# homopolymer/RAMBL

Measured on AMD Instinct MI355X. Metric: reads/sec into POA (150bp, ~1.5k-node graph), higher is better.
Workload: dtype f64

## Files before the change

### rambl_amd/csrc/sc_kernels.hip

```cpp
#include <hip/hip_runtime.h>
#include <math.h>
#include <stdint.h>
#include <stdlib.h>

#include "sc_device.hpp"

namespace sc {

#define SC_GLOBAL __attribute__((address_space(1)))
#define SC_LDS __attribute__((address_space(3)))

constexpr int LDS_TOTAL = 160 * 1024 - 256;
constexpr int LDS_SMALL = 18 * 1024;
constexpr int LDS_BIG = LDS_TOTAL - LDS_SMALL;
static_assert(LDS_SMALL >= (int)(sizeof(double) * 2 * MAXS + sizeof(StrainParam) * MAXS + sizeof(unsigned) * MAXS * KMAX + sizeof(int) * 6 * MAXS + 64), "LDS_SMALL");
static_assert(LDS_BIG >= (int)(sizeof(double) * MAXS * 64), "LDS_BIG");

template <int CTRL, int ROW_MASK, int BANK_MASK, bool BOUND>
__device__ __forceinline__ double dpp_f64(double v) {
    int lo = __double2loint(v), hi = __double2hiint(v);
    lo = __builtin_amdgcn_update_dpp(0, lo, CTRL, ROW_MASK, BANK_MASK, BOUND);
    hi = __builtin_amdgcn_update_dpp(0, hi, CTRL, ROW_MASK, BANK_MASK, BOUND);
    return __hiloint2double(hi, lo);
}
// ... 98 lines not shown
#pragma unroll
    for (int i = 0; i < NPL; i++) {
        const int s = lane * NPL + i;
        x[i] = -INFINITY;
        if (s < S) {
            const double* row = job.ll + (long)s_slot[s] * job.ll_stride;
            double v = hr ? row[rid] : 0.0;
            if (hu) v += row[uid];
            x[i] = v;
            m = fmax(m, v);
        }
    }
    for (int d = 1; d < 64; d <<= 1) m = fmax(m, __shfl_xor(m, d));
    const bool flag = !(m >= -600.0);
    double w[NPL], pair = 0;
#pragma unroll
    for (int i = 0; i < NPL; i++) {
        const int s = lane * NPL + i;
        w[i] = (s < S) ? a[i] * exp(x[i] - m) : 0.0;
        pair += w[i];
    }
    const double incl = wave_scan_incl(pair);
    const double T = readlane_f64(incl, 63);
    const double tgt = u * T;
    const double lo = tgt - DRAW_EPS64 * T, hi = tgt + DRAW_EPS64 * T;
    bool ok = (T > 0.0) && (T < 1.0e300) && !flag;
    int c;
    if (NPL == 1) {
        const unsigned long long mlo = __ballot(incl >= lo), mhi = __ballot(incl >= hi);
        ok = ok && (mlo == mhi) && (mlo != 0ull);
        c = ok ? (int)__builtin_ctzll(mlo) : 0;
    } else {
        const double E = wave_shr1(incl);
        const double c0 = E + w[0], c1 = E + pair;
        const unsigned long long m0lo = __ballot(c0 >= lo), m0hi = __ballot(c0 >= hi);
        const unsigned long long m1lo = __ballot(c1 >= lo), m1hi = __ballot(c1 >= hi);
        ok = ok && (m0lo == m0hi) && (m1lo == m1hi) && (m1lo != 0ull);
        const int l1 = ok ? (int)__builtin_ctzll(m1lo) : 0;
        c = 2 * l1 + (((m0lo >> l1) & 1ull) ? 0 : 1);
    }
    if (!ok) {
#pragma unroll
        for (int i = 0; i < NPL; i++) { int s = lane * NPL + i; if (s < S) s_a[s] = a[i]; }
        __builtin_amdgcn_wave_barrier();
        int cc = 0;
        if (lane == 0) cc = exact_draw(job, s_slot, s_a, s_p, S, rid, uid, u);
        c = __builtin_amdgcn_readfirstlane(cc);
        __builtin_amdgcn_wave_barrier();
        c |= 0x100;
    }
    return c;
}

typedef float f4v __attribute__((ext_vector_type(4)));
typedef float f2v __attribute__((ext_vector_type(2)));
typedef int i4v __attribute__((ext_vector_type(4)));
typedef unsigned u4v __attribute__((ext_vector_type(4)));

__device__ __forceinline__ float fma_rn(float a, float b, float c) {
    float d;
    asm("v_fma_f32 %0, %1, %2, %3" : "=v"(d) : "v"(a), "v"(b), "v"(c));
    return d;
}
__device__ __forceinline__ f2v pk_sub(f2v a, f2v b) {
    f2v d;
    asm("v_pk_add_f32 %0, %1, %2 neg_lo:[0,1] neg_hi:[0,1]" : "=v"(d) : "v"(a), "v"(b));
    return d;
}
__device__ __forceinline__ unsigned min3_u32(unsigned m, unsigned x, unsigned y) {
    unsigned d;
    asm("v_min3_u32 %0, %1, %2, %3" : "=v"(d) : "v"(m), "v"(x), "v"(y));
    return d;
}
template <int QP> __device__ __forceinline__ float quad_f32(float v) {
    return __int_as_float(__builtin_amdgcn_update_dpp(0, __float_as_int(v), QP, 0xF, 0xF, true));
}
template <int QP> __device__ __forceinline__ int quad_i32(int v) {
    return __builtin_amdgcn_update_dpp(0, v, QP, 0xF, 0xF, true);
}
__device__ __forceinline__ void lds_barrier() { asm volatile("s_waitcnt lgkmcnt(0)\n\ts_barrier" ::: "memory"); }

constexpr int UWIN = 1024;
#ifdef SC_CHAIN_PROF
__device__ unsigned long long g_chain_prof[12];
#define CHAIN_STAMP(k) do { if (wv == 0) { const unsigned long long t_ = clock64(); prof[k] += t_ - tprev; tprev = t_; } } while (0)
#define CHAIN_STAMP_W(k) do { asm volatile("s_waitcnt lgkmcnt(0)" ::: "memory"); CHAIN_STAMP(k); } while (0)
#else
#define CHAIN_STAMP(k) do {} while (0)
#define CHAIN_STAMP_W(k) do {} while (0)
#endif

template <int NQ, bool ROWS_LDS, int NW, class JD>
__device__ __forceinline__ void urn_chain_q(const JD& job, const LevelHdr& h, const StrainParam* s_sp, LevelResult* __restrict__ R,
                                            const int* s_slot, volatile double* s_a, volatile double* s_p, unsigned* s_kf,
                                            const float* s_a0f, int* s_x, float* s_uwin, const float* rows_lds, int stride, int tid) {
    constexpr int SPL = 4 * NQ, SP = 16 * NQ;
    constexpr int NPLC = SP > 64 ? 2 : 1;
    constexpr float EPSW = (float)(SP + 16) * 1.5e-7f;
    const int lane = tid & 63, wv = __builtin_amdgcn_readfirstlane(tid >> 6), k = lane & 3, pos = wv * 16 + (lane >> 2);
    const int S = h.S, Q = h.Q, n = h.n_sweeps, e0 = h.e0;
    const int Sm1 = S - 1;
    const int total = n * Q;
    const SlowArgs sa{job.qent, job.quid, job.ent_rid, job.ll, job.ll_stride, job.has};
    const SC_GLOBAL double* Ustream = (const SC_GLOBAL double*)job.U;
    const SC_GLOBAL float* Uf = (const SC_GLOBAL float*)job.Uf;
    const SC_GLOBAL float* rows_g = (const SC_GLOBAL float*)job.tabLf;
    SC_GLOBAL unsigned char* dlog = (SC_GLOBAL unsigned char*)job.dlog;
    auto ld4 = [&](int idx) __attribute__((always_inline)) -> f4v {
        return ROWS_LDS ? *(const f4v*)(rows_lds + idx) : *(const SC_GLOBAL f4v*)(rows_g + idx);
    };
    auto ld1 = [&](int idx) __attribute__((always_inline)) -> float { return ROWS_LDS ? rows_lds[idx] : rows_g[idx]; };

    const int cbase = k * SPL;
    const float m0 = k > 0 ? 1.0f : 0.0f, m1 = k > 1 ? 1.0f : 0.0f;
    const float posf = (float)pos + 1.0e-37f;
    double a0m[NPLC];
#pragma unroll
    for (int i = 0; i < NPLC; i++) { const int s = lane * NPLC + i; a0m[i] = (s < S) ? s_sp[s].a0 : 0.0; }
    f4v a0q[NQ];
#pragma unroll
    for (int g = 0; g < NQ; g++) a0q[g] = *(const f4v*)(s_a0f + cbase + 4 * g);
    unsigned long long n_exact = 0, n_slow = 0, n_pass = 0;
    const unsigned long long clk0 = clock64(), wall0 = wall_clock64();

    int ulo = 0;
    bool upf = false;
    f4v ux0 = 0.0f, ux1 = 0.0f;
    if (wv == 0) {
#pragma unroll
        for (int j = 0; j < UWIN / 256; j++) *(f4v*)(s_uwin + 256 * j + 4 * lane) = *(const SC_GLOBAL f4v*)(Uf + 256 * j + 4 * lane);
    }
    __syncthreads();

    int t = 0;
    int ro = (pos % Q) * stride;
    const int wrap = Q * stride;
    int upos = pos;
    f4v L[NQ];
    float uf = 0.0f, llast = 0.0f;
    auto issue_loads = [&]() __attribute__((always_inline)) {
#pragma unroll
        for (int g = 0; g < NQ; g++) L[g] = ld4(ro + cbase + 4 * g);
        llast = ld1(ro + Sm1);
        uf = s_uwin[upos];
    };
    if (total > 0) issue_loads();
#ifdef SC_CHAIN_PROF
    unsigned long long prof[9] = {0, 0, 0, 0, 0, 0, 0, 0, 0}, tprev = clock64();
#endif
#pragma unroll 1
    while (t < total) {
        asm volatile("" ::: "memory");
        n_pass++;
        float loc[SPL];
        float run = 0.0f;
        u4v kq[NQ];
#pragma unroll
        for (int g = 0; g < NQ; g++) kq[g] = *(const u4v*)(s_kf + cbase + 4 * g);
        const unsigned klast = s_kf[Sm1];
        const float a0last = s_a0f[Sm1];
#pragma unroll
        for (int g = 0; g < NQ; g++) {
            const u4v kk = kq[g];
            const f4v av = a0q[g] + f4v{(float)kk.x, (float)kk.y, (float)kk.z, (float)kk.w};
            loc[4 * g + 0] = run = (g == 0) ? av.x * L[g].x : fma_rn(av.x, L[g].x, run);
            loc[4 * g + 1] = run = fma_rn(av.y, L[g].y, run);
            loc[4 * g + 2] = run = fma_rn(av.z, L[g].z, run);
            loc[4 * g + 3] = run = fma_rn(av.w, L[g].w, run);
        }
        const float alast = a0last + (float)klast;
        CHAIN_STAMP(0);
        const float i1 = fmaf(quad_f32<0x90>(run), m0, run);
        const float i2 = fmaf(quad_f32<0x40>(i1), m1, i1);
        const float off = i2 - run;
        const float T = quad_f32<0xFF>(i2);
        const float tgt = uf * T;
        const float tb = tgt - off;
        const f2v tb2 = {tb, tb};
        unsigned w = 0;
        unsigned up = 0x7f800000u, dn = 0x7f800000u;
#pragma unroll
        for (int j = 0; j < SPL; j += 2) {
            const f2v lc = {loc[j], loc[j + 1]};
            const f2v d = pk_sub(lc, tb2);
            const f2v e = pk_sub(tb2, lc);
            w = __builtin_amdgcn_alignbit(w, __float_as_uint(d.x), 31);
            w = __builtin_amdgcn_alignbit(w, __float_as_uint(d.y), 31);
            up = min3_u32(up, __float_as_uint(d.x), __float_as_uint(d.y));
            dn = min3_u32(dn, __float_as_uint(e.x), __float_as_uint(e.y));
        }
        const float alt = tgt - (T - alast * llast);
        const float epsT = EPSW * T;
        const float lim_up = fmaf(uf + 0x1p-22f, posf, epsT);
        const float lim_dn = fmaf((1.0f + 0x1p-22f) - uf, posf, epsT);
        const bool okl = (__uint_as_float(dn) >= lim_dn) && ((__uint_as_float(up) >= lim_up) || (alt >= lim_dn));
        const unsigned long long F = ~__ballot(okl);
        const int fpos = F ? 16 * wv + ((int)__builtin_ctzll(F) >> 2) : 16 * NW;
        if (lane == 0) s_x[wv] = fpos;
        int c = __popc(w);
        c += quad_i32<0xB1>(c);
        c += quad_i32<0x4E>(c);
        c = min(c, Sm1);
        CHAIN_STAMP(1);
        lds_barrier();
        const int rem = total - t;
        int adv = 16 * NW;
#pragma unroll
        for (int j = 0; j < NW / 4; j++) {
            const i4v xf = *(const i4v*)(s_x + 4 * j);
            adv = min(adv, min(min(xf.x, xf.y), min(xf.z, xf.w)));
        }
        adv = adv < rem ? adv : rem;
        CHAIN_STAMP(2);
        if (adv == 0) {
            if (wv == 0) {
                const double u = Ustream[t];
                double ad[NPLC];
#pragma unroll
                for (int i = 0; i < NPLC; i++) { const int s = lane * NPLC + i; ad[i] = a0m[i] + (double)((s < S) ? s_kf[s] : 0u); }
                const int qi = __builtin_amdgcn_readfirstlane(ro) / stride;
                const int cc = slow_draw<NPLC>(sa, s_slot, s_a, s_p, ad[0], NPLC > 1 ? ad[NPLC - 1] : 0.0, S, qi, e0, u, lane);
                n_slow++;
                n_exact += (cc >> 8) & 1;
                c = cc & 0xFF;
            }
            adv = 1;
        }
        const bool acc = (pos < adv) && (k == 0);
        SC_GLOBAL unsigned char* const lg = dlog + (t + pos);
        t += adv;
        if (t >= total) {
            if (acc) { __hip_atomic_fetch_add(&s_kf[c], 1u, __ATOMIC_RELAXED, __HIP_MEMORY_SCOPE_WORKGROUP); *lg = (unsigned char)c; }
            break;
        }
        if (Q >= 16 * NW) {
            const unsigned r1 = (unsigned)(ro + adv * stride);
            const unsigned r2 = r1 - (unsigned)wrap;
            ro = (int)(r1 < r2 ? r1 : r2);
        } else {
            ro = ((ro / stride + adv) % Q) * stride;
        }
        upos = (upos + adv) & (UWIN - 1);
        if (wv == 0) {
            if (!upf && t >= ulo + UWIN / 4) {
                ux0 = *(const SC_GLOBAL f4v*)(Uf + ulo + UWIN + 4 * lane);
                ux1 = *(const SC_GLOBAL f4v*)(Uf + ulo + UWIN + 256 + 4 * lane);
                upf = true;
            }
            if (t >= ulo + UWIN / 2) {
                *(f4v*)(s_uwin + ((ulo & (UWIN - 1)) + 4 * lane)) = ux0;
                *(f4v*)(s_uwin + ((ulo & (UWIN - 1)) + 256 + 4 * lane)) = ux1;
                ulo += UWIN / 2;
                upf = false;
            }
        }
        CHAIN_STAMP(3);
        issue_loads();
        CHAIN_STAMP_W(6);
        if (acc) __hip_atomic_fetch_add(&s_kf[c], 1u, __ATOMIC_RELAXED, __HIP_MEMORY_SCOPE_WORKGROUP);
        CHAIN_STAMP_W(7);
        if (acc) *lg = (unsigned char)c;
        CHAIN_STAMP_W(8);
        lds_barrier();
        CHAIN_STAMP(4);
    }
#ifdef SC_CHAIN_PROF
    if (tid == 0) { for (int i = 0; i < 9; i++) if (i != 5) atomicAdd(&g_chain_prof[i], prof[i]); atomicAdd(&g_chain_prof[5], n_pass); }
#endif
    asm volatile("s_waitcnt vmcnt(0)" ::: "memory");
    __syncthreads();
    if (wv == 0) {
#pragma unroll
        for (int i = 0; i < NPLC; i++) {
            const int s = lane * NPLC + i;
            if (s < S) { R->abund[s] = a0m[i] + (double)s_kf[s]; R->kdraw[s] = s_kf[s]; }
        }
        if (lane == 0) {
            R->n_draws = (unsigned long long)total; R->n_exact = n_exact; R->n_slow = n_slow; R->n_pass = n_pass;
            R->chain_cycles = clock64() - clk0; R->chain_wall = wall_clock64() - wall0;
        }
    }
}

template <class JD>
__device__ __forceinline__ void draw_log_counts(const JD& job, const LevelHdr& h, unsigned* s_cnt, int tid, int nt) {
    const int Q = h.Q, n = h.n_sweeps;
    if (Q <= 0 || n <= 0) return;
    __builtin_amdgcn_fence(__ATOMIC_ACQUIRE, "agent");
    const SC_GLOBAL unsigned char* dlog = (const SC_GLOBAL unsigned char*)job.dlog;
    const int G = Q < nt ? min(nt / Q, n) : 1;
    const int per = (n + G - 1) / G;
    for (int idx = tid; idx < Q * G; idx += nt) {
        const int q = idx % Q, j0 = (idx / Q) * per, j1 = min(j0 + per, n);
        const int sym = job.qcode[q];
        if (sym >= KMAX || j0 >= j1) continue;
        const SC_GLOBAL unsigned char* p = dlog + (j0 * Q + q);
        int cur = 0;
        unsigned run = 0;
        auto count = [&](int c) __attribute__((always_inline)) {
            if (c != cur) {
                if (run) __hip_atomic_fetch_add(&s_cnt[cur * KMAX + sym], run, __ATOMIC_RELAXED, __HIP_MEMORY_SCOPE_WORKGROUP);
                cur = c; run = 0;
            }
            run++;
        };
        int j = j0;
        for (; j + 8 <= j1; j += 8, p += 8 * Q) {
            int c[8];
#pragma unroll
            for (int i = 0; i < 8; i++) c[i] = p[i * Q] & (MAXS - 1);
#pragma unroll
            for (int i = 0; i < 8; i++) count(c[i]);
        }
        for (; j < j1; j++, p += Q) count(*p & (MAXS - 1));
        if (run) __hip_atomic_fetch_add(&s_cnt[cur * KMAX + sym], run, __ATOMIC_RELAXED, __HIP_MEMORY_SCOPE_WORKGROUP);
    }
}

template <int NW>
__device__ __forceinline__ void urn_chain_shadow(const LevelHdr& h, const int* s_x) {
    const int total = h.n_sweeps * h.Q;
    __syncthreads();
    int t = 0;
#pragma unroll 1
    while (t < total) {
        lds_barrier();
        int adv = 16 * NW;
#pragma unroll
        for (int j = 0; j < NW / 4; j++) {
            const i4v xf = *(const volatile i4v*)(s_x + 4 * j);
            adv = min(adv, min(min(xf.x, xf.y), min(xf.z, xf.w)));
        }
        const int rem = total - t;
        adv = adv < rem ? adv : rem;
        if (adv == 0) adv = 1;
        t += adv;
        if (t >= total) break;
        lds_barrier();
    }
    __syncthreads();
}

enum { LV_COPIES_DONE = 1, LV_ITEMS_DONE = 2, LV_HAS_DONE = 4, LV_HARD_DONE = 8 };
typedef const __attribute__((address_space(4))) JobDev KJob;

__global__ __launch_bounds__(256) void k_level_copy(JobDev job, const LevelParams* __restrict__ P) {
    const int c = blockIdx.y;
    const double2* src = reinterpret_cast<const double2*>(job.ll + (long)P->copy_src[c] * job.ll_stride);
    double2* dst = reinterpret_cast<double2*>(job.ll + (long)P->copy_dst[c] * job.ll_stride);
    const int n2 = (job.n_reads + 1) >> 1;
    for (int i = blockIdx.x * blockDim.x + threadIdx.x; i < n2; i += gridDim.x * blockDim.x) dst[i] = src[i];
}

__global__ __launch_bounds__(256) void k_level_update(JobDev job, LevelHdr h, const LevelParams* __restrict__ P) {
    __shared__ double s_row[MAXS * KMAX];
    __shared__ double s_diag[MAXS * KMAX];
    __shared__ int s_slot[MAXS], s_lab[MAXS];
    const int tid = threadIdx.x;
    const int S = h.S, K = job.K, e0 = h.e0, Rn = h.e1 - h.e0, codeN = job.code_N;
    for (int s = tid; s < S; s += blockDim.x) { s_slot[s] = P->sp[s].slot; s_lab[s] = job.labels[P->sp[s].lab_off]; }
    __syncthreads();
    for (int i = tid; i < S * KMAX; i += blockDim.x) {
        const int sx = i / KMAX, b = i % KMAX, a = s_lab[sx];
        const double* lp = P->lpt + (long)sx * K * K;
        s_row[i] = (a < K && b < K) ? lp[a * K + b] : 0.0;
        s_diag[i] = (b < K) ? lp[b * K + b] : 0.0;
    }
    __syncthreads();
    const long total = (long)S * Rn;
    const long stride = job.ll_stride;
    for (long idx = (long)blockIdx.x * blockDim.x + tid; idx < total; idx += (long)gridDim.x * blockDim.x) {
        const int sx = (int)(idx / Rn), e = e0 + (int)(idx % Rn);
        const int rid = job.ent_rid[e];
        const int b = job.labels[job.ent_lab_off[e]];
        const bool fresh = job.ent_first[e] && !job.has[rid];
        if (sx == 0) job.isnew[e - e0] = fresh ? 1 : 0;
        int a = s_lab[sx];
        const bool wild = (a == codeN);
        if (wild) a = b;
        const double val = (a < K && b < K) ? (wild ? s_diag[sx * KMAX + b] : s_row[sx * KMAX + b]) : __longlong_as_double(0x7ff8000000000000ll);
        double* cell = job.ll + (long)s_slot[sx] * stride + rid;
        *cell = fresh ? val : (*cell + val);
    }
}

__global__ __launch_bounds__(256) void k_level_has(JobDev job, LevelHdr h) {
    const int Rn = h.e1 - h.e0;
    for (int r = blockIdx.x * blockDim.x + threadIdx.x; r < Rn; r += gridDim.x * blockDim.x) job.has[job.ent_rid[h.e0 + r]] = 1;
}

__global__ __launch_bounds__(256) void k_hard_slots(JobDev job, LevelHdr h) {
    const int e0 = h.e0, Rn = h.e1 - h.e0;
    for (int r = blockIdx.x * blockDim.x + threadIdx.x; r < Rn; r += gridDim.x * blockDim.x) {
        const int e = e0 + r;
        const int rid = job.ent_rid[e], cn = job.ent_cn[e];
        const int qb = job.ent_qoff[e];
        const int mb = job.mate_ptr[rid], mn = job.mate_ptr[rid + 1] - mb;
        const uint8_t code = (job.ent_lab_len[e] == 1) ? job.labels[job.ent_lab_off[e]] : (uint8_t)0xFF;
        for (int i = 0; i < cn; i++) {
            const int k = cn - 1 - i;
            job.qent[qb + i] = r;
            job.quid[qb + i] = (k < mn) ? job.mate_idx[mb + k] : -1;
            job.qcode[qb + i] = code;
        }
    }
}
__global__ __launch_bounds__(256) void k_hard_mates(JobDev job, LevelHdr h, const LevelParams* __restrict__ P) {
    const long stride = job.ll_stride;
    for (int q = blockIdx.x * blockDim.x + threadIdx.x; q < h.Q; q += gridDim.x * blockDim.x) {
        const int uid = job.quid[q];
// ... 176 lines not shown
            }
        }
    } else if (!h.has_dups) {
        const long total = (long)S * Rn;
        for (long idx = tid; idx < total; idx += nt) item((int)(idx / Rn), (int)(idx % Rn));
    } else {
        if (tid < S) for (int r = 0; r < Rn; r++) item(tid, r);
    }
    if (h.done & LV_HAS_DONE) { __syncthreads(); return; }
    __syncthreads();
    for (int r = tid; r < Rn; r += nt) job.has[job.ent_rid[e0 + r]] = 1;
    __syncthreads();
}

template <bool BARRIER = true, class JD>
__device__ __forceinline__ void phase_slots(const JD& job, const LevelHdr& h, int tid, int nt) {
    const int e0 = h.e0, Rn = h.e1 - h.e0;
    for (int r = tid; r < Rn; r += nt) {
        const int e = e0 + r;
        const int rid = job.ent_rid[e], cn = job.ent_cn[e];
        const int qb = job.ent_qoff[e];
        const int mb = job.mate_ptr[rid], mn = job.mate_ptr[rid + 1] - mb;
        const uint8_t code = (job.ent_lab_len[e] == 1) ? job.labels[job.ent_lab_off[e]] : (uint8_t)0xFF;
        for (int i = 0; i < cn; i++) {
            const int k = cn - 1 - i;
            const int uid = (k < mn) ? job.mate_idx[mb + k] : -1;
            job.qent[qb + i] = r;
            job.quid[qb + i] = uid;
            job.qcode[qb + i] = code;
        }
    }
    if (BARRIER) __syncthreads();
}

__device__ __forceinline__ void finish_level(const LevelHdr& h, LevelResult* __restrict__ R, unsigned long long wall0, int tid) {
    __threadfence_system();
    __syncthreads();
    if (tid == 0) {
        R->level_wall = wall_clock64() - wall0;
        R->xcc = (int)(__builtin_amdgcn_s_getreg(20 | (3 << 11)) & 0xF);
        R->xcc = (int)(__builtin_amdgcn_s_getreg(20 | (3 << 11)) & 0xF);
        __hip_atomic_store(&R->seq, h.seq, __ATOMIC_RELEASE, __HIP_MEMORY_SCOPE_SYSTEM);
    }
}

__device__ __forceinline__ float exp_weight(double y) {
    if (y < -104.0) return 0.0f;
    const double k = rint(y * 1.4426950408889634);
    double r = fma(k, -0.693147180559945286, y);
    r = fma(k, -2.3190468138462996e-17, r);
    const float e = __builtin_amdgcn_exp2f((float)r * 1.44269504f);
    const double kc = fmax(k, -300.0);
    return (y == y) ? ldexpf(e, (int)kc) : __int_as_float(0x7fc00000);
}

__host__ __device__ inline int chain_w_stride(int S) {
    const int s4 = (S + 1 + 3) & ~3;
    return (s4 & 4) ? s4 : s4 + 4;
}

struct LevelLds {
    double* s_a; double* s_p; unsigned* s_cnt; int* s_slot; unsigned* s_kf; float* s_a0f; int* s_x; int* s_copy; int* s_lab;
    StrainParam* s_sp; unsigned char* s_big;
};
__device__ __forceinline__ LevelLds level_lds(unsigned char* raw) {
    LevelLds l;
    l.s_a = reinterpret_cast<double*>(raw);
    l.s_p = l.s_a + MAXS;
    l.s_sp = reinterpret_cast<StrainParam*>(l.s_p + MAXS);
    l.s_cnt = reinterpret_cast<unsigned*>(l.s_sp + MAXS);
    l.s_slot = reinterpret_cast<int*>(l.s_cnt + MAXS * KMAX);
    l.s_kf = reinterpret_cast<unsigned*>(l.s_slot + MAXS);
    l.s_a0f = reinterpret_cast<float*>(l.s_kf + MAXS);
    l.s_copy = reinterpret_cast<int*>(l.s_a0f + MAXS);
    l.s_lab = l.s_copy + 2 * MAXS;
    l.s_x = l.s_lab + MAXS;
    l.s_big = raw + LDS_SMALL;
    return l;
}

constexpr int CHAINW_ROWS_BYTES = LDS_BIG - UWIN * 4;
constexpr int CHAIN_THREADS = 512;
constexpr int chain_nw(int nb) { return nb <= 2 ? 8 : 4; }
template <class IT>
__device__ __forceinline__ LevelHdr load_hdr(const IT& it) {
    LevelHdr h;
    h.mode = it.h.mode; h.S = it.h.S; h.e0 = it.h.e0; h.e1 = it.h.e1; h.has_dups = it.h.has_dups; h.any_multi = it.h.any_multi;
    h.Q = it.h.Q; h.n_sweeps = it.h.n_sweeps; h.n_copy = it.h.n_copy; h.do_update = it.h.do_update; h.done = it.h.done;
    h.copy_n = it.h.copy_n; h.seq = it.h.seq;
    return h;
}
template <int NB, bool ROWS_LDS, bool STAY, class IT>
__device__ __forceinline__ void level_sample_body(const IT& it, unsigned char* s_raw) {
    const unsigned long long wall0 = wall_clock64();
    const LevelHdr h = load_hdr(it);
    KJob& job = *(KJob*)it.job;
    const LevelParams* __restrict__ P = it.P;
    LevelResult* __restrict__ R = it.R;
    const LevelLds l = level_lds(s_raw);
    float* s_uwin = reinterpret_cast<float*>(l.s_big);
    float* s_rows = s_uwin + UWIN;
    const int tid = threadIdx.x;
    int nt = blockDim.x;
    const int S = h.S, Q = h.Q, e0 = h.e0, Rn = h.e1 - h.e0;
    const int stride = chain_w_stride(S);
    const bool upd = h.do_update && Rn > 0;
    stage_params(h, P, l.s_sp, l.s_copy, reinterpret_cast<double*>(l.s_big), upd && !(h.done & LV_ITEMS_DONE), job.K * job.K, tid, nt);
    for (int i = tid; i < MAXS * KMAX; i += nt) l.s_cnt[i] = 0;
    if (tid == 0) { R->error = 0; R->n_draws = 0; R->n_exact = 0; R->n_slow = 0; R->n_pass = 0; R->chain_cycles = 0; R->chain_wall = 0; }
    __syncthreads();
    if (tid == 0) R->phase_ticks[0] = (unsigned)(wall_clock64() - wall0);
    if (tid < MAXS) {
        l.s_slot[tid] = tid < S ? l.s_sp[tid].slot : 0;
        l.s_kf[tid] = 0u;
        l.s_a0f[tid] = tid < S ? (float)l.s_sp[tid].a0 : 0.0f;
        l.s_lab[tid] = tid < S ? (int)job.labels[l.s_sp[tid].lab_off] : 0;
    }
    phase_copies(job, h, l.s_copy, tid, nt);
    if (tid == 0) R->phase_ticks[1] = (unsigned)(wall_clock64() - wall0);
    if (upd) {
        phase_slots<false>(job, h, tid, nt);
        phase_update(job, h, l.s_sp, l.s_lab, reinterpret_cast<const double*>(l.s_big), tid, nt);
    }
    if (tid == 0) R->phase_ticks[2] = (unsigned)(wall_clock64() - wall0);
    if (!upd) phase_slots(job, h, tid, nt);
    if (tid == 0) R->phase_ticks[3] = (unsigned)(wall_clock64() - wall0);

    {
        constexpr int SR = (NB <= 2) ? 16 * NB : 16;
        const long lstride = job.ll_stride;
        SC_GLOBAL float* rows_g = (SC_GLOBAL float*)job.tabLf;
        auto put4 = [&](long idx, f4v v) __attribute__((always_inline)) {
            if (ROWS_LDS) *(f4v*)(s_rows + idx) = v; else *(SC_GLOBAL f4v*)(rows_g + idx) = v;
        };
        const float qnanf = __int_as_float(0x7fc00000);
        for (int q = tid; q < Q; q += nt) {
            const int rid = job.ent_rid[e0 + job.qent[q]], uid = job.quid[q];
            const bool hr = h.do_update ? true : job.has[rid] != 0;
            const bool hu = uid >= 0 && job.has[uid] != 0;
            const long Lf = (long)q * stride;
            auto cell = [&](int sx) __attribute__((always_inline)) -> double {
                const double* row = job.ll + (long)l.s_slot[sx] * lstride;
                double v = hr ? row[rid] : 0.0;
                if (hu) v += row[uid];
                return v;
            };
            double m = -INFINITY;
            double x[SR];
            if (NB <= 2) {
#pragma unroll
                for (int i = 0; i < SR; i++) { x[i] = -INFINITY; if (i < S) { x[i] = cell(i); m = fmax(m, x[i]); } }
            } else {
                for (int s0 = 0; s0 < S; s0 += SR) {
#pragma unroll
                    for (int i = 0; i < SR; i++) if (s0 + i < S) m = fmax(m, cell(s0 + i));
                }
            }
            const bool flag = !(m >= -600.0);
            for (int s0 = 0; s0 < stride; s0 += SR) {
                if (NB > 2) {
#pragma unroll
                    for (int i = 0; i < SR; i++) x[i] = (s0 + i < S) ? cell(s0 + i) : -INFINITY;
                }
#pragma unroll
                for (int i = 0; i < SR; i += 4) {
                    if (s0 + i < stride) {
                        f4v w;
#pragma unroll
                        for (int k = 0; k < 4; k++) {
                            const int sx = s0 + i + k;
                            const float wk = sx < S ? (flag ? qnanf : exp_weight(x[i + k] - m)) : 0.0f;
                            if (k == 0) w.x = wk; else if (k == 1) w.y = wk; else if (k == 2) w.z = wk; else w.w = wk;
                        }
                        put4(Lf + s0 + i, w);
                    }
                }
            }
            if (q == Q - 1) for (int i = 0; i < 16; i += 4) put4(Lf + stride + i, f4v{0.0f, 0.0f, 0.0f, 0.0f});
        }
    }
    __syncthreads();
    if (tid == 0) R->phase_ticks[4] = (unsigned)(wall_clock64() - wall0);
    constexpr int NW = chain_nw(NB);
    if (tid >= 64 * NW) {
        if (!STAY) return;
        urn_chain_shadow<NW>(h, l.s_x);
    } else {
        urn_chain_q<NB, ROWS_LDS, NW>(job, h, l.s_sp, R, l.s_slot, l.s_a, l.s_p, l.s_kf, l.s_a0f, l.s_x, s_uwin, s_rows, stride, tid);
    }
    if (!STAY) nt = 64 * NW;
    draw_log_counts(job, h, l.s_cnt, tid, nt);
    __syncthreads();
    for (int i = tid; i < S * KMAX; i += nt) R->cnt[i] = l.s_cnt[i];
    finish_level(h, R, wall0, tid);
}

template <class IT>
__device__ __forceinline__ void level_plain_body(const IT& it, unsigned char* s_raw) {
    const unsigned long long wall0 = wall_clock64();
    const LevelHdr h = load_hdr(it);
    KJob& job = *(KJob*)it.job;
    const LevelParams* __restrict__ P = it.P;
    LevelResult* __restrict__ R = it.R;
    const LevelLds l = level_lds(s_raw);
    double* s_tab = reinterpret_cast<double*>(l.s_big);
    const int tid = threadIdx.x, nt = blockDim.x;
    const int S = h.S, K = job.K, K2 = K * K, e0 = h.e0, Rn = h.e1 - h.e0;
    const long stride = job.ll_stride;
    const bool upd = h.do_update && Rn > 0;
    stage_params(h, P, l.s_sp, l.s_copy, s_tab, upd && !(h.done & LV_ITEMS_DONE), K2, tid, nt);
    if (tid == 0) { R->error = 0; R->n_draws = 0; R->n_exact = 0; R->n_slow = 0; R->n_pass = 0; R->chain_cycles = 0; R->chain_wall = 0; }
    __syncthreads();
    if (tid == 0) R->phase_ticks[0] = (unsigned)(wall_clock64() - wall0);
    if (tid < S) l.s_lab[tid] = (int)job.labels[l.s_sp[tid].lab_off];
    phase_copies(job, h, l.s_copy, tid, nt);
    if (tid == 0) R->phase_ticks[1] = (unsigned)(wall_clock64() - wall0);
    if (upd) phase_update(job, h, l.s_sp, l.s_lab, s_tab, tid, nt);
    if (tid == 0) R->phase_ticks[2] = (unsigned)(wall_clock64() - wall0);
    if (Rn <= 0 || S <= 0 || h.mode != MODE_HARD || (h.done & LV_HARD_DONE)) { finish_level(h, R, wall0, tid); return; }
    phase_slots(job, h, tid, nt);
    if (tid == 0) R->phase_ticks[3] = (unsigned)(wall_clock64() - wall0);

    const int Q = h.Q;
    for (int q = tid; q < Q; q += nt) {
        const int uid = job.quid[q];
        if (uid >= 0 && !job.has[uid])
            for (int s = 0; s < S; s++) job.ll[(long)l.s_sp[s].slot * stride + uid] = 0.0;
    }
    __syncthreads();
    for (int q = tid; q < Q; q += nt) { const int uid = job.quid[q]; if (uid >= 0) job.has[uid] = 1; }
    __syncthreads();
    for (long idx = tid; idx < (long)S * Q; idx += nt) {
        const int s = (int)(idx / Q), q = (int)(idx % Q);
        const int rid = job.ent_rid[e0 + job.qent[q]], uid = job.quid[q];
        const double* row = job.ll + (long)l.s_sp[s].slot * stride;
        double x = l.s_sp[s].logpri + row[rid];
        if (uid >= 0) x += row[uid];
        job.tabA[(long)s * job.qcap + q] = x;
    }
    __syncthreads();
    for (int q = tid; q < Q; q += nt) {
        const double* col = job.tabA + q;
        double m = -INFINITY;
        for (int s = 0; s < S; s++) m = fmax(m, col[(long)s * job.qcap]);
        double norm = 0;
        for (int s = 0; s < S; s++) norm += exp(col[(long)s * job.qcap] - m);
        for (int s = 0; s < S; s++) {
            double* cell = job.tabA + (long)s * job.qcap + q;
            *cell = exp(*cell - m) / norm;
        }
    }
    for (int i = tid; i < S * K2; i += nt) s_tab[i] = 0.0;
    __syncthreads();
    if (tid == 0) R->phase_ticks[4] = (unsigned)(wall_clock64() - wall0);
    if (!h.any_multi) {
        const int lane = tid & 63, wv = tid >> 6, nw = nt >> 6;
        for (int s = wv; s < S; s += nw) {
            const double* prow = job.tabA + (long)s * job.qcap;
            double acc[KMAX + 1];
#pragma unroll
            for (int b = 0; b <= KMAX; b++) acc[b] = 0.0;
            for (int q = lane; q < Q; q += 64) {
                const double p = prow[q];
                const int code = job.qcode[q];
                acc[KMAX] += p;
#pragma unroll
                for (int b = 0; b < KMAX; b++) acc[b] += (code == b) ? p : 0.0;
            }
#pragma unroll
            for (int b = 0; b <= KMAX; b++) {
                double v = acc[b];
// ... 541 lines not shown
            done |= LV_HARD_DONE;
        }
    }
    return done;
}
int level_kind(const LevelHdr& h) {
    const int S = h.S, Q = h.Q, Rn = h.e1 - h.e0;
    const bool chain = h.mode == MODE_SAMPLE && h.n_sweeps > 0 && S > 1 && Rn > 0;
    if (!chain) return 0;
    const bool wl = ((long)Q * chain_w_stride(S) + 16) * 4 <= (long)CHAINW_ROWS_BYTES;
    int nb = (S + 15) / 16;
    nb = nb < 1 ? 1 : (nb > 8 ? 8 : nb);
    return 1 + 2 * (nb - 1) + (wl ? 1 : 0);
}
int level_lds_kb(const LevelHdr& h, int K) {
    const int kind = level_kind(h);
    const long S = h.S, Rn = h.e1 - h.e0;
    long big = 0;
    if ((h.do_update && Rn > 0) || h.mode == MODE_HARD) big = (long)sizeof(double) * S * K * K;
    if (kind != 0) {
        long rows = (long)UWIN * 4;
        if ((kind - 1) & 1) rows += ((long)h.Q * chain_w_stride(h.S) + 16) * 4;
        if (rows > big) big = rows;
    }
    long need = LDS_SMALL + big + 64;
    if (need > LDS_TOTAL) need = LDS_TOTAL;
    return (int)((need + 1023) / 1024);
}
static size_t batch_lds(const LevelBatch& b, int n) {
    int kb = 0;
    for (int i = 0; i < n; i++) { const int k = (b.it[i].kind >> 8) & 0xFFFF; kb = k > kb ? k : kb; }
    size_t bytes = (size_t)kb * 1024;
    if (kb == 0 || bytes > (size_t)LDS_TOTAL) bytes = LDS_TOTAL;
    return bytes;
}
void launch_level_any(hipStream_t st, const LevelBatch& b, int n) {
    hipLaunchKernelGGL(k_level_any, dim3(n), dim3(CHAIN_THREADS), batch_lds(b, n), st, b);
}
void launch_level_batch(hipStream_t st, int kind, const LevelBatch& b, int n) {
    const size_t lds = batch_lds(b, n);
    if (kind == 0) {
        hipLaunchKernelGGL(k_level, dim3(n), dim3(512), lds, st, b);
        return;
    }
    const bool wl = (kind - 1) & 1;
#define SC_SAMPLE(NB) case NB: if (wl) hipLaunchKernelGGL((k_level_sample<NB, true>), dim3(n), dim3(CHAIN_THREADS), lds, st, b); \
                               else hipLaunchKernelGGL((k_level_sample<NB, false>), dim3(n), dim3(CHAIN_THREADS), lds, st, b); break;
    switch ((kind - 1) / 2 + 1) {
        SC_SAMPLE(1) SC_SAMPLE(2) SC_SAMPLE(3) SC_SAMPLE(4) SC_SAMPLE(5) SC_SAMPLE(6) SC_SAMPLE(7)
        default: if (wl) hipLaunchKernelGGL((k_level_sample<8, true>), dim3(n), dim3(CHAIN_THREADS), lds, st, b);
                 else hipLaunchKernelGGL((k_level_sample<8, false>), dim3(n), dim3(CHAIN_THREADS), lds, st, b);
    }
#undef SC_SAMPLE
}
void launch_resident(hipStream_t st, const ResidentArgs& a, int slots) {
    hipLaunchKernelGGL(k_level_resident, dim3(slots), dim3(CHAIN_THREADS), CHAIN_LDS, st, a);
}
void launch_msa(hipStream_t st, const MsaDev& d) {
    if (d.cmax > MSA_CM || d.mv_stride > 64) hipLaunchKernelGGL(k_msa<true>, dim3(1), dim3(256), 0, st, d);
    else hipLaunchKernelGGL(k_msa<false>, dim3(1), dim3(256), MSA_LDS, st, d);
}
void launch_thread(hipStream_t st, const ThreadDev& d, int* pool_sorted) {
    const int ncls = d.glen * 8;
    int blocks = (d.n_reads + 3) / 4;
    if (blocks > 2048) blocks = 2048;
    if (blocks < 1) blocks = 1;
    hipLaunchKernelGGL((k_thread_walk<false>), dim3(blocks), dim3(256), 0, st, d);
    hipLaunchKernelGGL(k_thread_scan, dim3(1), dim3(1024), 0, st, d.count, d.off, ncls);
    hipLaunchKernelGGL((k_thread_walk<true>), dim3(blocks), dim3(256), 0, st, d);
    int sblocks = (ncls + 3) / 4;
    if (sblocks > 2048) sblocks = 2048;
    hipLaunchKernelGGL(k_thread_sort, dim3(sblocks), dim3(256), 0, st, d.off, d.pool, pool_sorted, ncls, d.big);
    static const int big_words = [] {
        const char* e = getenv("SC_SORT_BIG_WORDS");
        const int w = e ? atoi(e) : BIG_WORDS;
        return w < 64 ? 64 : (w > BIG_WORDS ? BIG_WORDS : w);
    }();
    if (d.n_reads > SORT_WORDS * 32)
        hipLaunchKernelGGL(k_thread_sort_big, dim3(512), dim3(1024), BIG_WORDS * 8, st, d.off, d.pool, pool_sorted, d.big, big_words);
}

}
#ifdef SC_CHAIN_PROF
extern "C" int sc_debug_chain_prof(unsigned long long* out) {
    return (int)hipMemcpyFromSymbol(out, HIP_SYMBOL(sc::g_chain_prof), sizeof(unsigned long long) * 12);
}
#endif
```

Before: 15050.

## Process two draw positions per quad in urn chain for mid-size strain counts

Adds a DPL template parameter so each lane group evaluates two consecutive draw positions per pass when NB is 3-5, doubling the speculative window of the sequential urn chain per barrier round. The aim is to amortize the per-pass LDS barrier and ballot/fpos reduction over more draws and give more ILP to the prefix-sum and threshold checks. The cost is more registers and loads per pass and more wasted speculative work when an early position fails. The profiling counters are also split per NQ kind.

After: 14110. 0.938x the previous value.

```diff
diff --git a/rambl_amd/csrc/sc_kernels.hip b/rambl_amd/csrc/sc_kernels.hip
--- a/rambl_amd/csrc/sc_kernels.hip
+++ b/rambl_amd/csrc/sc_kernels.hip
@@ -204,7 +204,7 @@
 
 constexpr int UWIN = 1024;
 #ifdef SC_CHAIN_PROF
-__device__ unsigned long long g_chain_prof[12];
+__device__ unsigned long long g_chain_prof[24];
 #define CHAIN_STAMP(k) do { if (wv == 0) { const unsigned long long t_ = clock64(); prof[k] += t_ - tprev; tprev = t_; } } while (0)
 #define CHAIN_STAMP_W(k) do { asm volatile("s_waitcnt lgkmcnt(0)" ::: "memory"); CHAIN_STAMP(k); } while (0)
 #else
@@ -212,14 +212,15 @@
 #define CHAIN_STAMP_W(k) do {} while (0)
 #endif
 
-template <int NQ, bool ROWS_LDS, int NW, class JD>
+template <int NQ, bool ROWS_LDS, int NW, int DPL, class JD>
 __device__ __forceinline__ void urn_chain_q(const JD& job, const LevelHdr& h, const StrainParam* s_sp, LevelResult* __restrict__ R,
                                             const int* s_slot, volatile double* s_a, volatile double* s_p, unsigned* s_kf,
                                             const float* s_a0f, int* s_x, float* s_uwin, const float* rows_lds, int stride, int tid) {
     constexpr int SPL = 4 * NQ, SP = 16 * NQ;
+    constexpr int W = 16 * NW * DPL;
     constexpr int NPLC = SP > 64 ? 2 : 1;
     constexpr float EPSW = (float)(SP + 16) * 1.5e-7f;
-    const int lane = tid & 63, wv = __builtin_amdgcn_readfirstlane(tid >> 6), k = lane & 3, pos = wv * 16 + (lane >> 2);
+    const int lane = tid & 63, wv = __builtin_amdgcn_readfirstlane(tid >> 6), k = lane & 3, pos = wv * (16 * DPL) + (lane >> 2);
     const int S = h.S, Q = h.Q, n = h.n_sweeps, e0 = h.e0;
     const int Sm1 = S - 1;
     const int total = n * Q;
@@ -235,7 +236,9 @@
 
     const int cbase = k * SPL;
     const float m0 = k > 0 ? 1.0f : 0.0f, m1 = k > 1 ? 1.0f : 0.0f;
-    const float posf = (float)pos + 1.0e-37f;
+    float posf[DPL];
+#pragma unroll
+    for (int d = 0; d < DPL; d++) posf[d] = (float)(pos + 16 * d) + 1.0e-37f;
     double a0m[NPLC];
 #pragma unroll
     for (int i = 0; i < NPLC; i++) { const int s = lane * NPLC + i; a0m[i] = (s < S) ? s_sp[s].a0 : 0.0; }
@@ -255,16 +258,23 @@
     __syncthreads();
 
     int t = 0;
-    int ro = (pos % Q) * stride;
+    int ro[DPL];
     const int wrap = Q * stride;
     int upos = pos;
-    f4v L[NQ];
-    float uf = 0.0f, llast = 0.0f;
+    f4v L[DPL][NQ];
+    float uf[DPL], llast[DPL];
+#pragma unroll
+    for (int d = 0; d < DPL; d++) { ro[d] = ((pos + 16 * d) % Q) * stride; uf[d] = 0.0f; llast[d] = 0.0f; }
     auto issue_loads = [&]() __attribute__((always_inline)) {
 #pragma unroll
-        for (int g = 0; g < NQ; g++) L[g] = ld4(ro + cbase + 4 * g);
-        llast = ld1(ro + Sm1);
-        uf = s_uwin[upos];
+        for (int g = 0; g < NQ; g++)
+#pragma unroll
+            for (int d = 0; d < DPL; d++) L[d][g] = ld4(ro[d] + cbase + 4 * g);
+#pragma unroll
+        for (int d = 0; d < DPL; d++) {
+            llast[d] = ld1(ro[d] + Sm1);
+            uf[d] = s_uwin[(upos + 16 * d) & (UWIN - 1)];
+        }
     };
     if (total > 0) issue_loads();
 #ifdef SC_CHAIN_PROF
@@ -274,8 +284,8 @@
     while (t < total) {
         asm volatile("" ::: "memory");
         n_pass++;
-        float loc[SPL];
-        float run = 0.0f;
+        float loc[DPL][SPL];
+        float run[DPL];
         u4v kq[NQ];
 #pragma unroll
         for (int g = 0; g < NQ; g++) kq[g] = *(const u4v*)(s_kf + cbase + 4 * g);
@@ -285,48 +295,74 @@
         for (int g = 0; g < NQ; g++) {
             const u4v kk = kq[g];
             const f4v av = a0q[g] + f4v{(float)kk.x, (float)kk.y, (float)kk.z, (float)kk.w};
-            loc[4 * g + 0] = run = (g == 0) ? av.x * L[g].x : fma_rn(av.x, L[g].x, run);
-            loc[4 * g + 1] = run = fma_rn(av.y, L[g].y, run);
-            loc[4 * g + 2] = run = fma_rn(av.z, L[g].z, run);
-            loc[4 * g + 3] = run = fma_rn(av.w, L[g].w, run);
+#pragma unroll
+            for (int d = 0; d < DPL; d++) loc[d][4 * g + 0] = run[d] = (g == 0) ? av.x * L[d][g].x : fma_rn(av.x, L[d][g].x, run[d]);
+#pragma unroll
+            for (int d = 0; d < DPL; d++) loc[d][4 * g + 1] = run[d] = fma_rn(av.y, L[d][g].y, run[d]);
+#pragma unroll
+            for (int d = 0; d < DPL; d++) loc[d][4 * g + 2] = run[d] = fma_rn(av.z, L[d][g].z, run[d]);
+#pragma unroll
+            for (int d = 0; d < DPL; d++) loc[d][4 * g + 3] = run[d] = fma_rn(av.w, L[d][g].w, run[d]);
         }
         const float alast = a0last + (float)klast;
         CHAIN_STAMP(0);
-        const float i1 = fmaf(quad_f32<0x90>(run), m0, run);
-        const float i2 = fmaf(quad_f32<0x40>(i1), m1, i1);
-        const float off = i2 - run;
-        const float T = quad_f32<0xFF>(i2);
-        const float tgt = uf * T;
-        const float tb = tgt - off;
-        const f2v tb2 = {tb, tb};
-        unsigned w = 0;
-        unsigned up = 0x7f800000u, dn = 0x7f800000u;
+        float i1[DPL], i2[DPL], T[DPL], tgt[DPL];
+        f2v tb2[DPL];
+#pragma unroll
+        for (int d = 0; d < DPL; d++) i1[d] = fmaf(quad_f32<0x90>(run[d]), m0, run[d]);
+#pragma unroll
+        for (int d = 0; d < DPL; d++) i2[d] = fmaf(quad_f32<0x40>(i1[d]), m1, i1[d]);
+#pragma unroll
+        for (int d = 0; d < DPL; d++) T[d] = quad_f32<0xFF>(i2[d]);
+#pragma unroll
+        for (int d = 0; d < DPL; d++) {
+            const float off = i2[d] - run[d];
+            tgt[d] = uf[d] * T[d];
+            const float tb = tgt[d] - off;
+            tb2[d] = f2v{tb, tb};
+        }
+        unsigned w[DPL], up[DPL], dn[DPL];
+#pragma unroll
+        for (int d = 0; d < DPL; d++) { w[d] = 0; up[d] = 0x7f800000u; dn[d] = 0x7f800000u; }
 #pragma unroll
         for (int j = 0; j < SPL; j += 2) {
-            const f2v lc = {loc[j], loc[j + 1]};
-            const f2v d = pk_sub(lc, tb2);
-            const f2v e = pk_sub(tb2, lc);
-            w = __builtin_amdgcn_alignbit(w, __float_as_uint(d.x), 31);
-            w = __builtin_amdgcn_alignbit(w, __float_as_uint(d.y), 31);
-            up = min3_u32(up, __float_as_uint(d.x), __float_as_uint(d.y));
-            dn = min3_u32(dn, __float_as_uint(e.x), __float_as_uint(e.y));
-        }
-        const float alt = tgt - (T - alast * llast);
-        const float epsT = EPSW * T;
-        const float lim_up = fmaf(uf + 0x1p-22f, posf, epsT);
-        const float lim_dn = fmaf((1.0f + 0x1p-22f) - uf, posf, epsT);
-        const bool okl = (__uint_as_float(dn) >= lim_dn) && ((__uint_as_float(up) >= lim_up) || (alt >= lim_dn));
-        const unsigned long long F = ~__ballot(okl);
-        const int fpos = F ? 16 * wv + ((int)__builtin_ctzll(F) >> 2) : 16 * NW;
+#pragma unroll
+            for (int d = 0; d < DPL; d++) {
+                const f2v lc = {loc[d][j], loc[d][j + 1]};
+                const f2v df = pk_sub(lc, tb2[d]);
+                const f2v e = pk_sub(tb2[d], lc);
+                w[d] = __builtin_amdgcn_alignbit(w[d], __float_as_uint(df.x), 31);
+                w[d] = __builtin_amdgcn_alignbit(w[d], __float_as_uint(df.y), 31);
+                up[d] = min3_u32(up[d], __float_as_uint(df.x), __float_as_uint(df.y));
+                dn[d] = min3_u32(dn[d], __float_as_uint(e.x), __float_as_uint(e.y));
+            }
+        }
+        unsigned long long F[DPL];
+        int cd[DPL];
+#pragma unroll
+        for (int d = 0; d < DPL; d++) {
+            const float alt = tgt[d] - (T[d] - alast * llast[d]);
+            const float epsT = EPSW * T[d];
+            const float lim_up = fmaf(uf[d] + 0x1p-22f, posf[d], epsT);
+            const float lim_dn = fmaf((1.0f + 0x1p-22f) - uf[d], posf[d], epsT);
+            const bool okl = (__uint_as_float(dn[d]) >= lim_dn) && ((__uint_as_float(up[d]) >= lim_up) || (alt >= lim_dn));
+            F[d] = ~__ballot(okl);
+            int cc = __popc(w[d]);
+            cc += quad_i32<0xB1>(cc);
+            cc += quad_i32<0x4E>(cc);
+            cd[d] = min(cc, Sm1);
+        }
+        int fpos = W;
+#pragma unroll
+        for (int d = DPL - 1; d >= 0; d--) fpos = F[d] ? 16 * (DPL * wv + d) + ((int)__builtin_ctzll(F[d]) >> 2) : fpos;
         if (lane == 0) s_x[wv] = fpos;
-        int c = __popc(w);
-        c += quad_i32<0xB1>(c);
-        c += quad_i32<0x4E>(c);
-        c = min(c, Sm1);
+        int c = cd[0];
+        if (DPL > 1) c = (k == 1) ? cd[DPL - 1] : c;
+        const int cpos = pos + ((DPL > 1 && k == 1) ? 16 : 0);
         CHAIN_STAMP(1);
         lds_barrier();
         const int rem = total - t;
-        int adv = 16 * NW;
+        int adv = W;
 #pragma unroll
         for (int j = 0; j < NW / 4; j++) {
             const i4v xf = *(const i4v*)(s_x + 4 * j);
@@ -340,7 +376,7 @@
                 double ad[NPLC];
 #pragma unroll
                 for (int i = 0; i < NPLC; i++) { const int s = lane * NPLC + i; ad[i] = a0m[i] + (double)((s < S) ? s_kf[s] : 0u); }
-                const int qi = __builtin_amdgcn_readfirstlane(ro) / stride;
+                const int qi = __builtin_amdgcn_readfirstlane(ro[0]) / stride;
                 const int cc = slow_draw<NPLC>(sa, s_slot, s_a, s_p, ad[0], NPLC > 1 ? ad[NPLC - 1] : 0.0, S, qi, e0, u, lane);
                 n_slow++;
                 n_exact += (cc >> 8) & 1;
@@ -348,19 +384,24 @@
             }
             adv = 1;
         }
-        const bool acc = (pos < adv) && (k == 0);
-        SC_GLOBAL unsigned char* const lg = dlog + (t + pos);
+        const bool acc = (cpos < adv) && (k < DPL);
+        SC_GLOBAL unsigned char* const lg = dlog + (t + cpos);
         t += adv;
         if (t >= total) {
             if (acc) { __hip_atomic_fetch_add(&s_kf[c], 1u, __ATOMIC_RELAXED, __HIP_MEMORY_SCOPE_WORKGROUP); *lg = (unsigned char)c; }
             break;
         }
-        if (Q >= 16 * NW) {
-            const unsigned r1 = (unsigned)(ro + adv * stride);
-            const unsigned r2 = r1 - (unsigned)wrap;
-            ro = (int)(r1 < r2 ? r1 : r2);
+        if (Q >= W) {
+            const unsigned step = (unsigned)(adv * stride);
+#pragma unroll
+            for (int d = 0; d < DPL; d++) {
+                const unsigned r1 = (unsigned)ro[d] + step;
+                const unsigned r2 = r1 - (unsigned)wrap;
+                ro[d] = (int)(r1 < r2 ? r1 : r2);
+            }
         } else {
-            ro = ((ro / stride + adv) % Q) * stride;
+#pragma unroll
+            for (int d = 0; d < DPL; d++) ro[d] = ((ro[d] / stride + adv) % Q) * stride;
         }
         upos = (upos + adv) & (UWIN - 1);
         if (wv == 0) {
@@ -387,7 +428,11 @@
         CHAIN_STAMP(4);
     }
 #ifdef SC_CHAIN_PROF
-    if (tid == 0) { for (int i = 0; i < 9; i++) if (i != 5) atomicAdd(&g_chain_prof[i], prof[i]); atomicAdd(&g_chain_prof[5], n_pass); }
+    if (tid == 0) {
+        unsigned long long* gp = g_chain_prof + (NQ > 2 ? 12 : 0);
+        for (int i = 0; i < 9; i++) if (i != 5) atomicAdd(&gp[i], prof[i]);
+        atomicAdd(&gp[5], n_pass);
+    }
 #endif
     asm volatile("s_waitcnt vmcnt(0)" ::: "memory");
     __syncthreads();
@@ -439,7 +484,7 @@
     }
 }
 
-template <int NW>
+template <int NW, int DPL>
 __device__ __forceinline__ void urn_chain_shadow(const LevelHdr& h, const int* s_x) {
     const int total = h.n_sweeps * h.Q;
     __syncthreads();
@@ -447,7 +492,7 @@
 #pragma unroll 1
     while (t < total) {
         lds_barrier();
-        int adv = 16 * NW;
+        int adv = 16 * NW * DPL;
 #pragma unroll
         for (int j = 0; j < NW / 4; j++) {
             const i4v xf = *(const volatile i4v*)(s_x + 4 * j);
@@ -790,6 +835,7 @@
 constexpr int CHAINW_ROWS_BYTES = LDS_BIG - UWIN * 4;
 constexpr int CHAIN_THREADS = 512;
 constexpr int chain_nw(int nb) { return nb <= 2 ? 8 : 4; }
+constexpr int chain_dpl(int nb) { return (nb >= 3 && nb <= 5) ? 2 : 1; }
 template <class IT>
 __device__ __forceinline__ LevelHdr load_hdr(const IT& it) {
     LevelHdr h;
@@ -889,12 +935,12 @@
     }
     __syncthreads();
     if (tid == 0) R->phase_ticks[4] = (unsigned)(wall_clock64() - wall0);
-    constexpr int NW = chain_nw(NB);
+    constexpr int NW = chain_nw(NB), DPL = chain_dpl(NB);
     if (tid >= 64 * NW) {
         if (!STAY) return;
-        urn_chain_shadow<NW>(h, l.s_x);
+        urn_chain_shadow<NW, DPL>(h, l.s_x);
     } else {
-        urn_chain_q<NB, ROWS_LDS, NW>(job, h, l.s_sp, R, l.s_slot, l.s_a, l.s_p, l.s_kf, l.s_a0f, l.s_x, s_uwin, s_rows, stride, tid);
+        urn_chain_q<NB, ROWS_LDS, NW, DPL>(job, h, l.s_sp, R, l.s_slot, l.s_a, l.s_p, l.s_kf, l.s_a0f, l.s_x, s_uwin, s_rows, stride, tid);
     }
     if (!STAY) nt = 64 * NW;
     draw_log_counts(job, h, l.s_cnt, tid, nt);
@@ -1602,7 +1648,13 @@
 
 }
 #ifdef SC_CHAIN_PROF
+extern "C" int sc_debug_chain_prof_kinds(unsigned long long* out) {
+    return (int)hipMemcpyFromSymbol(out, HIP_SYMBOL(sc::g_chain_prof), sizeof(unsigned long long) * 24);
+}
 extern "C" int sc_debug_chain_prof(unsigned long long* out) {
-    return (int)hipMemcpyFromSymbol(out, HIP_SYMBOL(sc::g_chain_prof), sizeof(unsigned long long) * 12);
+    unsigned long long v[24];
+    const int rc = sc_debug_chain_prof_kinds(v);
+    for (int i = 0; i < 12; i++) out[i] = v[i] + v[12 + i];
+    return rc;
 }
 #endif
```
